# roljon/Steered-Mixture-of-Experts

Hardware: NVIDIA B200
Metric: pixel_kernel_evals_per_s_fwd_bwd (higher is better)
Workload: dtype f32

## Files before the change

### include/smoe_b200.h

```cpp
#ifndef SMOE_B200_H
#define SMOE_B200_H

#include <stddef.h>
#include <stdint.h>

#ifdef __cplusplus
extern "C" {
#endif

#define SMOE_ABI_VERSION 4
#define SMOE_TPIX 512
#define SMOE_NSCAL 16

#define SMOE_PIXEL_ABSENT (-1.0f)
#define SMOE_PIXEL_HALO   (-2.0f)

#define SMOE_E_BADARG (-1)
#define SMOE_E_UNSUPPORTED (-2)

typedef struct smoe_cfg {
    int32_t d;
    int32_t C;
    int32_t precision;
    float   margin;
    int32_t use_determinant;
// ... 56 lines not shown
                  uint8_t* infl_clear , int K_all, void* stream);

int smoe_spatial_keys(const float* centres, int K, int d, int row_stride, const float* grid ,
                      const float* scale , long long* keys, void* stream);

int smoe_forward(const smoe_cfg* cfg, const smoe_batch* batch, const float* packed, const int32_t* indices,
                 const int32_t* counts, const float* chunk_bounds, int K_cap, const float* loss_weights,
                 const float* ax0, const float* ax1, const float* ax2, float* rbuf, int32_t* argmax, uint8_t* infl,
                 float* pix, float* tile_qmin , unsigned long long* pair_counts, void* stream);

int smoe_loss_partials(const smoe_batch* batch);
int smoe_loss(const smoe_cfg* cfg, const smoe_batch* batch, const float* rbuf, const float* image,
              const uint8_t* image_u8, const float* loss_weights, float* res, float* pix, float* scalars,
              float* partials, int32_t* ticket, void* stream);

int smoe_cotangent(const smoe_cfg* cfg, const smoe_batch* batch, const float* rbuf, const float* grad_r, float* pix,
                   void* stream);

int smoe_backward(const smoe_cfg* cfg, const smoe_batch* batch, const float* packed, const int32_t* counts,
                  int K_cap, const float* pix, const float* tile_qmin,
                  const float* ax0, const float* ax1, const float* ax2, int num_splits, float* raw_part,
                  int32_t* plan ,
                  unsigned long long* pair_counts , void* stream);
size_t smoe_backward_plan_bytes(int K_cap, const smoe_batch* batch);
int smoe_suggest_splits(int K_cap, const smoe_batch* batch);

int smoe_reduce_splits(const smoe_cfg* cfg, const int32_t* counts, int K_cap, int num_splits,
                       const float* raw_part, const int32_t* plan ,
                       float* raw, void* stream);

// ... 82 lines not shown
```

### steered-mixture-of-experts_b200/_ffi.py

```python
from __future__ import annotations

import ctypes as C
import os

import torch

_HERE = os.path.dirname(os.path.abspath(__file__))
LIB_PATH = os.path.join(_HERE, "libsmoe_b200.so")

TPIX = 512
ABI_VERSION = 4
NSCAL = 16
STATS_STRIDE = 24

EXPORTS = [
    "smoe_abi_version", "smoe_last_error", "smoe_param_count", "smoe_packed_stride", "smoe_num_tiles", "smoe_pix_stride",
    "smoe_pack_workspace_bytes", "smoe_backward_workspace_bytes", "smoe_backward_plan_bytes", "smoe_pack", "smoe_pack_fed", "smoe_forward", "smoe_loss", "smoe_loss_partials", "smoe_cotangent", "smoe_ssim_loss_workspace_bytes", "smoe_ssim_loss",
    "smoe_backward", "smoe_suggest_splits", "smoe_reduce_splits", "smoe_grad_finalize", "smoe_update_kernel_list",
    "smoe_adam_step", "smoe_step_begin", "smoe_spatial_keys", "smoe_xchg_window_bytes", "smoe_peer_alloc", "smoe_peer_free",
    "smoe_peer_export", "smoe_peer_open", "smoe_peer_close", "smoe_xchg_publish", "smoe_grad_finalize_peers",
    "smoe_xchg_reduce_tail", "smoe_xchg_status", "smoe_feed", "smoe_halo_pull", "smoe_quant_ranges_bytes", "smoe_quant_ranges", "smoe_quant_route", "smoe_fake_quant_theta", "smoe_ssim_workspace_bytes", "smoe_ssim", "smoe_sqerr", "smoe_quantize", "smoe_rescale",
    "smoe_colminmax",
]


class Cfg(C.Structure):
    _fields_ = [("d", C.c_int32), ("C", C.c_int32), ("precision", C.c_int32), ("margin", C.c_float),
                ("use_determinant", C.c_int32), ("train_inverse_cov", C.c_int32), ("use_yuv", C.c_int32),
                ("train_gammas", C.c_int32), ("only_y_gamma", C.c_int32), ("quantize_pis", C.c_int32),
                ("pis_lb", C.c_float), ("pis_ub", C.c_float), ("pis_bits", C.c_int32),
                ("quantization_mode", C.c_int32), ("q_lb", C.c_float * 5), ("q_ub", C.c_float * 5),
                ("q_bits", C.c_int32 * 5), ("use_diff_center", C.c_int32), ("kernel_count_as_norm_l1", C.c_int32),
# ... 76 lines not shown
```

### steered-mixture-of-experts_b200/csrc/forward.cu

```cuda
#include "smoe_common.cuh"

namespace smoe {

template <int D, int C>
struct Rec {
    static constexpr int T = tri(D);
    static constexpr int GN = T + D + 1;
    static constexpr int EN = C + D * C;
    static constexpr int RC0 = (GN + EN + 1 + 3) / 4 * 4;
    static constexpr int RC = (RC0 / 4) % 2 == 0 ? RC0 + 4 : RC0;
    static constexpr int NG4 = (GN + 3) / 4;
    static constexpr int OQ = 0, OL = T, OC = T + D, ONU = GN, OGA = GN + C, OK = GN + EN;
};

template <int D, int C>
__device__ __forceinline__ void transform_record(const float* __restrict__ raw, const float (&mu)[D],
                                                 const float (&ctr)[3], int korig, float* __restrict__ dst) {
    using R = Rec<D, C>;
    float out[R::RC];
    float Qm[D][D], v[D];
#pragma unroll
    for (int l = 0; l < D; ++l)
#pragma unroll
        for (int m = l; m < D; ++m) Qm[l][m] = Qm[m][l] = raw[off_A(D, C) + ut(D, l, m)];
// ... 36 lines not shown
__device__ __forceinline__ void parabola(const float* __restrict__ f, const float (&xs)[3], float& c, float& b) {
    using R = Rec<D, C>;
    c = f[R::OC];
#pragma unroll
    for (int l = 1; l < D; ++l) {
        float t = f[R::OL + l];
#pragma unroll
        for (int m = l; m < D; ++m) t = fmaf(f[R::OQ + ut(D, l, m)], xs[m], t);
        c = fmaf(t, xs[l], c);
    }
    b = f[R::OL + 0];
#pragma unroll
    for (int m = 1; m < D; ++m) b = fmaf(f[R::OQ + ut(D, 0, m)], xs[m], b);
}

struct FwdArgs {
    smoe_cfg cfg;
    smoe_batch b;
    const float* packed;
    const int32_t* indices;
    const int32_t* counts;
    const float* chunk_bounds;
    const float* lossw;
    const float* ax[3];
    float* rbuf;
    int32_t* argmax;
    uint8_t* infl;
    float* pix;
    float* tile_qmin;
    unsigned long long* pair_counts;
    int ntiles, nt1, nt2, max_chunks;
    float tau, ltau;
    float eps_cut;
// ... 16 lines not shown
    *total = tot;
    return off + __popc(bal & ((1u << lane) - 1u));
}

#ifndef SMOE_FWD_CTAS_2D
#define SMOE_FWD_CTAS_2D 6
#endif
#ifndef SMOE_FWD_UNROLL
#define SMOE_FWD_UNROLL 2
#endif
constexpr int kBodyUnroll = SMOE_FWD_UNROLL;
#ifndef SMOE_FWD_NEARCUT
#define SMOE_FWD_NEARCUT 8.0f
#endif
constexpr float kNearCut = SMOE_FWD_NEARCUT;
template <int D, int C, bool COUNT, bool AMAX>
__global__ void __launch_bounds__(kThreadsF, (D == 2) ? SMOE_FWD_CTAS_2D : 4) forward_kernel(const FwdArgs a) {
    using R = Rec<D, C>;
    constexpr int PK = pstride(D, C);
    constexpr int PPT = kPixPerThread;
    static_assert(kChunk == kThreadsF, "one kernel of a chunk per thread");
    extern __shared__ __align__(128) unsigned char smem_raw[];
    float* raw0 = reinterpret_cast<float*>(smem_raw);
    float* raw1 = raw0 + kChunk * PK;
    float* crec = raw1 + kChunk * PK;
    uint64_t* bar = reinterpret_cast<uint64_t*>(crec + kChunk * R::RC);
    float* red = reinterpret_cast<float*>(bar + 2);
    int* scratch = reinterpret_cast<int*>(red + 32);
    int* clist = scratch + 8;

    const int tid = threadIdx.x;
    const int K = a.counts[0];
    const int nchunks = (K + kChunk - 1) / kChunk;
    const int mode = a.cfg.dense_exec;
    const bool cull = mode == 0, skip = mode != 1;
    if (tid == 0) {
        mbar_init(&bar[0], 1);
        mbar_init(&bar[1], 1);
        fence_barrier_init();
    }
    __syncthreads();
    uint32_t phase0 = 0, phase1 = 0;
    int par = 0;
// ... 33 lines not shown
            auto in_halo = [&](int ax, int g) {
                const int o = a.b.origin[ax], e = o + a.b.extent[ax];
                return ax < D && ((o > 0 && g < o + a.b.halo) || (e < a.b.dims[ax] && g >= e - a.b.halo));
            };
            const bool h12 = a.b.halo > 0 && (in_halo(1, g1) || in_halo(2, g2));
            if (D > 1) xs[1] = a.ax[1][min(g1, hi[1])] - ctr[1];
            if (D > 2) xs[2] = a.ax[2][min(g2, hi[2])] - ctr[2];
#pragma unroll
            for (int p = 0; p < PPT; ++p) {
                const int j = p * kThreadsF + tid;
                const int i0 = j / (e2 * e1);
                const int g0 = lo[0] + i0;
                const bool ok = g0 <= hi[0] && g1 <= hi[1] && g2 <= hi[2];
                bool fed = ok;
                if (a.lossw && ok && a.lossw[g0 * a.b.dims[1] * a.b.dims[2] + gbase12] == SMOE_PIXEL_ABSENT) fed = false;
                if (fed) okmask |= 1u << p;
                if (a.b.halo > 0 && (h12 || in_halo(0, g0))) hmask |= 1u << p;
                x0[p] = a.ax[0][min(g0, hi[0])] - ctr[0];
            }
        }

        auto build_chunk_list = [&](float thr, int part) -> int {
            int n = 0;
            for (int base = 0; base < nchunks; base += kThreadsF) {
                const int ci = base + tid;
                bool need = false;
                if (ci < nchunks) {
                    const float* cb = a.chunk_bounds + (size_t)ci * kCB;
                    float d2 = 0.f, kd = 0.f;
#pragma unroll
// ... 182 lines not shown
                    }
#pragma unroll
                    for (int p = 0; p < PPT; ++p) {
                        const float w = ex2f(q[p]);
                        const bool pass = q[p] > ltau;
                        const float wm = pass ? w : 0.f;
#pragma unroll
                        for (int c = 0; c < C; ++c) r[p][c] = fmaf(wm, fmaf(f[R::OGA + c], x0[p], Eb[c]), r[p][c]);
                        if (AMAX && pass && (w > bestw[p] || (w == bestw[p] && korig < bestk[p]))) { bestw[p] = w; bestk[p] = korig; }
                    }
                    if (any && a.infl) a.infl[korig] = 1;
                }
            });
        }

#pragma unroll
        for (int p = 0; p < PPT; ++p) {
            const int j = p * kThreadsF + tid;
            const bool inb = (okmask >> p) & 1u;
            const int gpix = (lo[0] + j / (e2 * e1)) * a.b.dims[1] * a.b.dims[2] + gbase12;
            const bool halo = ((hmask >> p) & 1u) || (a.lossw && inb && a.lossw[gpix] == SMOE_PIXEL_HALO);
            if (inb && !halo) {
#pragma unroll
                for (int c = 0; c < C; ++c) a.rbuf[(size_t)gpix * C + c] = r[p][c];
                if (AMAX) a.argmax[gpix] = bestk[p];
            }
            if (a.pix) {
                const int RLf = a.b.tile[D - 1];
                float* tp = a.pix + (size_t)tile * pix_stride(D, C, RLf);
                tp[PL_Z * SMOE_TPIX + j] = D == 1 ? x0[p] : xs[D - 1];
                tp[PL_QTHR * SMOE_TPIX + j] = inb ? qthr[p] : INFINITY;
                tp[PL_GR * SMOE_TPIX + j] = (inb && ((live_mask >> p) & 1u)) ? 1.f : 0.f;
                if (D > 1 && j % RLf == 0) {
                    const int row = j / RLf, nrows = SMOE_TPIX / RLf;
                    tp[pix_rowc_offset(C) + row] = x0[p];
#pragma unroll
                    for (int l = 1; l < D - 1; ++l) tp[pix_rowc_offset(C) + l * nrows + row] = xs[l];
                }
            }
        }
    }

    if (COUNT) {
        unsigned long long v[4] = {cntA_vis, cntA_ex, cntB_vis, cntB_ex};
#pragma unroll
        for (int q = 0; q < 4; ++q) {
#pragma unroll
            for (int o = 16; o > 0; o >>= 1) v[q] += __shfl_down_sync(0xffffffffu, v[q], o);
            if ((tid & 31) == 0) atomicAdd(&a.pair_counts[q], v[q]);
        }
    }

}

struct LossArgs {
    smoe_cfg cfg;
    smoe_batch b;
    const float* rbuf;
    const float* image;
    const uint8_t* image_u8;
    const float* lossw;
    float* res;
    float* pix;
    float* scalars;
    float* partials;
    int32_t* ticket;
    int ntiles, nt1, nt2, pix_tstride;
    float eps, q_scale, q_inv_scale;
};

template <int C>
__global__ void __launch_bounds__(256) loss_kernel(const LossArgs a) {
    const int tid = threadIdx.x;
    const int e1 = a.b.tile[1], e2 = a.b.tile[2];
    const int D = a.cfg.d;
    float lsum[C];
#pragma unroll
    for (int c = 0; c < C; ++c) lsum[c] = 0.f;
    float sqsum = 0.f;
    int nonfinite = 0;
    {
        int tt[3], lo[3], hi[3];
        tt[0] = blockIdx.y;
        tt[1] = a.nt2 == 1 ? (int)blockIdx.x : (int)blockIdx.x / a.nt2;
        tt[2] = a.nt2 == 1 ? 0 : (int)blockIdx.x % a.nt2;
        const int tile = (tt[0] * a.nt1 + tt[1]) * a.nt2 + tt[2];
#pragma unroll
        for (int i = 0; i < 3; ++i) {
            lo[i] = a.b.origin[i] + tt[i] * a.b.tile[i];
            hi[i] = min(lo[i] + a.b.tile[i], a.b.origin[i] + a.b.extent[i]) - 1;
        }
        auto in_halo = [&](int ax, int g) {
            const int o = a.b.origin[ax], e = o + a.b.extent[ax];
            return ax < D && ((o > 0 && g < o + a.b.halo) || (e < a.b.dims[ax] && g >= e - a.b.halo));
        };
// ... 2 lines not shown
        const int g1 = lo[1] + i1, g2 = lo[2] + i2;
        const bool in12 = g1 <= hi[1] && g2 <= hi[2];
        const bool halo12 = a.b.halo > 0 && (in_halo(1, g1) || in_halo(2, g2));
        const int rows_per_pass = 256 / (e1 * e2);
        int g0 = lo[0] + tid / (e1 * e2);
        for (int j = tid; j < SMOE_TPIX; j += 256, g0 += rows_per_pass) {
            bool inb = in12 && g0 <= hi[0];
            const int gpix = inb ? (g0 * a.b.dims[1] + g1) * a.b.dims[2] + g2 : 0;
            const float lwv = (a.lossw && inb) ? a.lossw[gpix] : 1.f;
            if (lwv == SMOE_PIXEL_ABSENT) inb = false;
            const bool halo = lwv == SMOE_PIXEL_HALO || halo12 || (a.b.halo > 0 && in_halo(0, g0));
            float g[C], gr = 0.f;
#pragma unroll
            for (int c = 0; c < C; ++c) g[c] = 0.f;
            if (inb && !halo) {
#pragma unroll
                for (int c = 0; c < C; ++c) {
                    const size_t gi = (size_t)gpix * C + c;
                    const float rv = a.rbuf[gi];
                    if (!(fabsf(rv) <= 3.0e38f)) nonfinite = 1;
                    const float rc = fminf(fmaxf(rv, 0.f), 1.f);
                    const float kq = floorf(__fadd_rn(__fmul_rn(rc, a.q_inv_scale), 0.5f));
                    const float rq = __fmul_rn(kq, a.q_scale);
                    const float tgt = a.image_u8 ? __fdiv_rn((float)a.image_u8[gi], 255.0f) : a.image[gi];
                    const float diff = __fsub_rn(rq, tgt);
                    const float ad = fabsf(diff) - a.eps;
                    sqsum = fmaf(diff, diff, sqsum);
                    lsum[c] = a.lossw ? fmaf(ad * ad, lwv, lsum[c]) : fmaf(ad, ad, lsum[c]);
                    const float cw = a.cfg.use_yuv ? (c == 0 ? 0.75f : 0.125f) : (1.0f / C);
                    const float sgn = diff > 0.f ? 1.f : (diff < 0.f ? -1.f : 0.f);
                    const bool ste = (rv >= 0.f) && (rv <= 1.f);
                    g[c] = ste ? 2.f * ad * sgn * cw * a.b.inv_count : 0.f;
                    if (a.lossw) g[c] *= lwv;
                    gr = fmaf(g[c], rv, gr);
                    if (a.res) a.res[gi] = rq;
                }
            }
            if (tp) {
                const bool live = tp[PL_GR * SMOE_TPIX + j] != 0.f;
                tp[PL_GR * SMOE_TPIX + j] = live ? gr : 0.f;
#pragma unroll
                for (int c = 0; c < C; ++c) tp[(PL_G + c) * SMOE_TPIX + j] = g[c];
            }
        }
    }
    __shared__ float red[8][8];
    __shared__ float tree[256];
    __shared__ int s_last;
    const int nblk = gridDim.x * gridDim.y, bid = blockIdx.y * gridDim.x + blockIdx.x;
    float vals[8];
#pragma unroll
    for (int q = 0; q < 8; ++q) vals[q] = 0.f;
#pragma unroll
    for (int c = 0; c < C; ++c) vals[c] = lsum[c];
    vals[4] = sqsum;
    vals[5] = (float)nonfinite;
#pragma unroll
    for (int q = 0; q < 6; ++q)
#pragma unroll
        for (int o = 16; o > 0; o >>= 1) vals[q] += __shfl_down_sync(0xffffffffu, vals[q], o);
    if ((tid & 31) == 0)
#pragma unroll
        for (int q = 0; q < 8; ++q) red[tid >> 5][q] = vals[q];
    __syncthreads();
    if (tid < 8) {
        float s = 0.f;
        for (int wv = 0; wv < 8; ++wv) s += red[wv][tid];
        a.partials[(size_t)bid * 8 + tid] = s;
    }
    __threadfence();
    __syncthreads();
    if (tid == 0) s_last = (atomicAdd(a.ticket, 1) == nblk - 1);
    __syncthreads();
    if (s_last) {
        __threadfence();
        for (int q = 0; q < 6; ++q) {
            float s = 0.f;
            for (int bq = tid; bq < nblk; bq += 256) s += __ldcg(&a.partials[(size_t)bq * 8 + q]);
            tree[tid] = s;
            __syncthreads();
            for (int o = 128; o > 0; o >>= 1) {
                if (tid < o) tree[tid] += tree[tid + o];
                __syncthreads();
            }
            if (tid == 0) a.scalars[q] += tree[0];
            __syncthreads();
        }
        if (tid == 0) *a.ticket = 0;
    }
}

struct CotArgs {
    smoe_batch b;
    const float* rbuf;
    const float* grad_r;
    float* pix;
    int nt1, nt2, pix_tstride;
};

template <int C>
__global__ void __launch_bounds__(256) cotangent_kernel(const CotArgs a) {
    const int tid = threadIdx.x;
    const int e1 = a.b.tile[1], e2 = a.b.tile[2];
// ... 24 lines not shown
            for (int c = 0; c < C; ++c) {
                const size_t gi = (size_t)gpix * C + c;
                g[c] = a.grad_r[gi];
                gr = fmaf(g[c], a.rbuf[gi], gr);
            }
        }
        const bool live = tp[PL_GR * SMOE_TPIX + j] != 0.f;
        tp[PL_GR * SMOE_TPIX + j] = live ? gr : 0.f;
#pragma unroll
        for (int c = 0; c < C; ++c) tp[(PL_G + c) * SMOE_TPIX + j] = g[c];
    }
}

template <int D, int C>
static size_t fwd_smem_bytes(int max_chunks) {
    return (size_t)(2 * kChunk * pstride(D, C) + kChunk * Rec<D, C>::RC) * 4 + 2 * 8 + 32 * 4 + 8 * 4 +
           (size_t)max_chunks * 4 + 64;
}

}

using namespace smoe;

extern "C" int smoe_forward(const smoe_cfg* cfg, const smoe_batch* batch, const float* packed, const int32_t* indices,
                            const int32_t* counts, const float* chunk_bounds, int K_cap, const float* loss_weights,
                            const float* ax0, const float* ax1, const float* ax2, float* rbuf, int32_t* argmax,
                            uint8_t* infl, float* pix, float* tile_qmin, unsigned long long* pair_counts, void* stream) {
    SMOE_REQUIRE(cfg && batch && packed && indices && counts && chunk_bounds && ax0 && ax1 && rbuf, "null argument");
    SMOE_REQUIRE(K_cap > 0, "K_cap must be positive");
    SMOE_REQUIRE(cfg->d == 2 || ax2, "ax2 required for d == 3");
    SMOE_REQUIRE(batch->tile[0] * batch->tile[1] * batch->tile[2] == SMOE_TPIX, "tile product must be SMOE_TPIX");
    SMOE_REQUIRE(kThreadsF % (batch->tile[1] * batch->tile[2]) == 0 && batch->tile[cfg->d - 1] % 4 == 0,
                 "tile[1]*tile[2] must divide 128 and the last tile extent must be a multiple of 4");
    SMOE_REQUIRE(!pix || tile_qmin, "tile_qmin is required with pix");
    SMOE_REQUIRE(batch->halo >= 0, "negative halo");
    SMOE_REQUIRE(cfg->eps_bits == 0 || (cfg->eps_bits >= 24 && cfg->eps_bits <= 126), "eps_bits must be 0 or in [24, 126]");
    SMOE_REQUIRE(cfg->eps_bits == 0 || cfg->dense_exec == 0, "eps_bits needs dense_exec == 0");
    for (int i = 0; i < 3; ++i)
        SMOE_REQUIRE(batch->extent[i] > 0 && batch->origin[i] >= 0 && batch->origin[i] + batch->extent[i] <= batch->dims[i],
                     "batch rectangle outside the image");
    SMOE_REQUIRE(cfg->d == 3 || (batch->dims[2] == 1 && batch->tile[2] == 1), "d == 2 needs dims[2] == tile[2] == 1");
    SMOE_REQUIRE((long long)batch->dims[0] * batch->dims[1] * batch->dims[2] < (1ll << 31), "more than 2^31 pixels");
// ... 6 lines not shown
    a.rbuf = rbuf; a.argmax = argmax; a.infl = infl; a.pix = pix; a.tile_qmin = tile_qmin;
    a.pair_counts = pair_counts;
    a.nt1 = (batch->extent[1] + batch->tile[1] - 1) / batch->tile[1];
    a.nt2 = (batch->extent[2] + batch->tile[2] - 1) / batch->tile[2];
    a.ntiles = smoe_num_tiles(batch);
    a.max_chunks = (K_cap + kChunk - 1) / kChunk;
    const float two_p = (float)(1 << cfg->precision);
    a.tau = 0.5f / two_p;
    a.ltau = -(float)(cfg->precision + 1);
    a.eps_cut = (float)cfg->eps_bits;
    int dev = 0, sms = 0;
    cudaGetDevice(&dev);
    cudaDeviceGetAttribute(&sms, cudaDevAttrMultiProcessorCount, dev);
    const int per_sm = cfg->d == 2 ? SMOE_FWD_CTAS_2D : 4;
    int grid = a.ntiles < per_sm * sms ? a.ntiles : per_sm * sms;
    cudaStream_t st = (cudaStream_t)stream;
#define LAUNCH(D, C, CNT, AM)                                                                                       \
    {                                                                                                               \
        size_t sm = fwd_smem_bytes<D, C>(a.max_chunks);                                                             \
        SMOE_REQUIRE(sm <= 200 * 1024, "too many kernel chunks for the shared-memory chunk list");                  \
        cudaFuncSetAttribute(forward_kernel<D, C, CNT, AM>, cudaFuncAttributeMaxDynamicSharedMemorySize, (int)sm);  \
        forward_kernel<D, C, CNT, AM><<<grid, kThreadsF, sm, st>>>(a);                                              \
    }
#define CALL(D, C)                                                               \
    if (pair_counts) { if (argmax) LAUNCH(D, C, true, true) else LAUNCH(D, C, true, false) } \
    else { if (argmax) LAUNCH(D, C, false, true) else LAUNCH(D, C, false, false) }
    SMOE_DISPATCH_DC(cfg->d, cfg->C, CALL)
#undef CALL
#undef LAUNCH
    return check_launch("smoe_forward");
}

extern "C" int smoe_loss_partials(const smoe_batch* batch) {
    return batch ? smoe_num_tiles(batch) : 0;
}

extern "C" int smoe_loss(const smoe_cfg* cfg, const smoe_batch* batch, const float* rbuf, const float* image,
                         const uint8_t* image_u8, const float* loss_weights, float* res, float* pix, float* scalars,
                         float* partials, int32_t* ticket, void* stream) {
    SMOE_REQUIRE(cfg && batch && rbuf && scalars && partials && ticket, "null argument");
    SMOE_REQUIRE((image != nullptr) != (image_u8 != nullptr), "exactly one of image / image_u8");
    SMOE_REQUIRE(batch->tile[0] * batch->tile[1] * batch->tile[2] == SMOE_TPIX, "tile product must be SMOE_TPIX");
    SMOE_REQUIRE(cfg->C == 1 || cfg->C == 3, "1 or 3 channels");
    SMOE_REQUIRE(256 % (batch->tile[1] * batch->tile[2]) == 0, "tile[1]*tile[2] must divide 256");
    LossArgs a;
    a.cfg = *cfg;
    a.b = *batch;
    a.rbuf = rbuf; a.image = image; a.image_u8 = image_u8; a.lossw = loss_weights; a.res = res; a.pix = pix;
    a.scalars = scalars; a.partials = partials; a.ticket = ticket;
    a.nt1 = (batch->extent[1] + batch->tile[1] - 1) / batch->tile[1];
    a.nt2 = (batch->extent[2] + batch->tile[2] - 1) / batch->tile[2];
    a.ntiles = smoe_num_tiles(batch);
    a.pix_tstride = pix_stride(cfg->d, cfg->C, batch->tile[cfg->d - 1]);
    const float two_p = (float)(1 << cfg->precision);
    a.eps = cfg->margin / two_p;
    a.q_scale = 1.0f / (two_p - 1.0f);
    a.q_inv_scale = 1.0f / a.q_scale;
    const int nt0 = a.ntiles / (a.nt1 * a.nt2);
    SMOE_REQUIRE(nt0 <= 65535, "too many tiles along the first axis");
    const dim3 grid(a.nt1 * a.nt2, nt0);
    if (cfg->C == 1) loss_kernel<1><<<grid, 256, 0, (cudaStream_t)stream>>>(a);
    else loss_kernel<3><<<grid, 256, 0, (cudaStream_t)stream>>>(a);
    return check_launch("smoe_loss");
}

extern "C" int smoe_cotangent(const smoe_cfg* cfg, const smoe_batch* batch, const float* rbuf, const float* grad_r,
                              float* pix, void* stream) {
    SMOE_REQUIRE(cfg && batch && rbuf && grad_r && pix, "null argument");
    SMOE_REQUIRE(batch->tile[0] * batch->tile[1] * batch->tile[2] == SMOE_TPIX, "tile product must be SMOE_TPIX");
    SMOE_REQUIRE(batch->halo == 0, "halo must be 0: the cotangent covers the whole batch rectangle");
    SMOE_REQUIRE((cfg->d == 2 || cfg->d == 3) && (cfg->C == 1 || cfg->C == 3), "d in {2, 3} and 1 or 3 channels");
    SMOE_REQUIRE(256 % (batch->tile[1] * batch->tile[2]) == 0, "tile[1]*tile[2] must divide 256");
// ... 14 lines not shown
```

### steered-mixture-of-experts_b200/csrc/smoe_common.cuh

```cuda
#pragma once
#include <cuda_runtime.h>
#include <stdint.h>
#include <stdio.h>
#include <math.h>
#include "../../include/smoe_b200.h"

#if defined(__CUDA_ARCH__) && (__CUDA_ARCH__ < 1000)
#error "libsmoe_b200 is written for sm_100a (B200) only"
#endif

namespace smoe {

#ifndef SMOE_BWD_THREADS
#define SMOE_BWD_THREADS 64
#endif
#ifndef SMOE_BWD_HALVES
#define SMOE_BWD_HALVES 2
#endif
constexpr int kThreads = SMOE_BWD_THREADS;
constexpr int kHalves = SMOE_BWD_HALVES;
constexpr int kGroup = kThreads / kHalves;
constexpr int kFin = 64;
constexpr int kThreadsF = 128;
constexpr int kPixPerThread = SMOE_TPIX / kThreadsF;
// ... 92 lines not shown
    for (int sp = 0; sp < used; sp += 8) {
        float v[8];
#pragma unroll
        for (int u = 0; u < 8; ++u) v[u] = (sp + u < used) ? p[(size_t)(sp + u) * stride] : 0.f;
#pragma unroll
        for (int u = 0; u < 8; ++u)
            if (sp + u < used) acc += v[u];
    }
    return acc;
}
__device__ __forceinline__ float ex2f(float x) {
    float y;
    asm("ex2.approx.ftz.f32 %0, %1;" : "=f"(y) : "f"(x));
    return y;
}
__device__ __forceinline__ uint32_t smem_u32(const void* p) {
    return (uint32_t)__cvta_generic_to_shared(p);
}
__device__ __forceinline__ void mbar_init(uint64_t* bar, uint32_t count) {
    asm volatile("mbarrier.init.shared::cta.b64 [%0], %1;" ::"r"(smem_u32(bar)), "r"(count));
}
__device__ __forceinline__ void fence_barrier_init() {
    asm volatile("fence.mbarrier_init.release.cluster;" ::: "memory");
}
__device__ __forceinline__ void fence_proxy_async() {
    asm volatile("fence.proxy.async.shared::cta;" ::: "memory");
}
__device__ __forceinline__ void mbar_expect_tx(uint64_t* bar, uint32_t bytes) {
    asm volatile("mbarrier.arrive.expect_tx.shared::cta.b64 _, [%0], %1;" ::"r"(smem_u32(bar)), "r"(bytes)
                 : "memory");
// ... 25 lines not shown
```

### steered-mixture-of-experts_b200/smoe.py

```python
from __future__ import annotations

import ctypes as C
import math
from itertools import product

import numpy as np
import torch

import os
import warnings

from . import _ffi
from ._ffi import Adam, Batch, Cfg, Peers, check, lib, ptr, stream_ptr
from .quantizer import quantize_params, rescaler

PARAM_KEYS = ("pis", "musX", "A_diagonal", "A_corr", "gamma_e", "nu_e")


def theta_offsets(d, C):
    T = d * (d + 1) // 2
    return dict(mu=0, A=d, pi=d + T, nu=d + T + 1, ga=d + T + 1 + C)


def a_col(d, l, m):
# ... 683 lines not shown
                self._graphs[key] = "warm"
            else:
                if state == "warm":
                    l0 = self.gpu_launches
                    if self._img_pending:
                        torch.cuda.current_stream().wait_event(self._img_event)
                        self._img_pending = False
                    torch.cuda.synchronize()
                    try:
                        graphs = []
                        for phase in (("pre", "post") if len(self._batches) == 1 else ()):
                            g = torch.cuda.CUDAGraph()
                            with torch.cuda.graph(g):
                                self._enqueue(pis_l1, u_l1, True, False, False, lossw=lossw, phase=phase)
                            graphs.append(g)
                        gall = torch.cuda.CUDAGraph()
                        with torch.cuda.graph(gall):
                            self._enqueue(pis_l1, u_l1, True, False, False, lossw=lossw)
                        state = (gall, graphs, (self.gpu_launches - l0) // (2 if graphs else 1))
                    except Exception as exc:
                        if os.environ.get("SMOE_ALLOW_EAGER", "0") != "1":
                            raise RuntimeError(f"smoe_b200: CUDA graph capture of the training step failed ({exc}); "
                                               "set SMOE_ALLOW_EAGER=1 to run the step eagerly instead") from exc
                        warnings.warn(f"smoe_b200: CUDA graph capture failed ({exc}); running eagerly")
                        self.use_cuda_graphs = False
                        torch.cuda.synchronize()
                        state = None
                    self.gpu_launches = l0
                    if state is not None:
                        self._graphs[key] = state
                if state is not None:
                    if self._img_pending and state[1]:
                        state[1][0].replay()
                        torch.cuda.current_stream().wait_event(self._img_event)
                        self._img_pending = False
                        state[1][1].replay()
                    else:
                        if self._img_pending:
                            torch.cuda.current_stream().wait_event(self._img_event)
                            self._img_pending = False
                        state[0].replay()
                    self.gpu_launches += state[2]
                    replayed = True
        if not replayed:
            self._enqueue(pis_l1, u_l1, train, update_reconstruction, with_quantized_params,
                          lossw=lossw, batches=batches)
        torch.cuda.current_stream().synchronize()
        h = self._host_f32.tolist()
        hi = self._host_i32.tolist()
        for row, irow in zip(h, hi):
            row[_ffi.NSCAL:_ffi.NSCAL + 4] = irow[_ffi.NSCAL:_ffi.NSCAL + 4]
        norm = float(self.start_pis)
        Cc = self.image.shape[-1]
        loss_val = mse_val = 0.0
        num_pi = -1
        for ii, b in enumerate(batches):
            inv_n = float(b.inv_count)
# ... 101 lines not shown
            rp = {k: torch.as_tensor(np.ascontiguousarray(np.asarray(v, dtype=np.float32)), device=self.device)
                  for k, v in self.rparams.items()}
            Kf = int(rp["pis"].shape[0])
            if Kf > K:
                raise ValueError("more fed kernels than model kernels")
            fkeys = torch.empty((Kf,), dtype=torch.int64, device=self.device)
            check(L.smoe_spatial_keys(ptr(rp["musX"]), Kf, self.dim_domain, self.dim_domain, ptr(None), self._key_scale,
                                      ptr(fkeys), st), "smoe_spatial_keys")
            forder = torch.sort(fkeys, stable=True).indices.to(torch.int32)
        norm = float(self.start_pis)
        if pre and self._qdyn is not None and not fed:
            check(L.smoe_quant_ranges(C.byref(self._cfg), ptr(self._theta), K, int(self.train_musx), ptr(self._qdyn), st),
                  "smoe_quant_ranges")
            self.gpu_launches += 2
        ax2 = ptr(self._d_axes[2]) if self.dim_domain == 3 else ptr(None)
        for ii, b in enumerate(batches):
            counts, regs, scal = self._counts[ii], self._regsums[ii], self._scalars[ii]
            tq = self._tile_qmin[ii]
            if pre:
                if fed:
                    check(L.smoe_pack_fed(C.byref(self._cfg), ptr(rp["A"]), ptr(rp["musX"]), ptr(rp["nu_e"]),
                                          ptr(rp["gamma_e"]), ptr(rp["pis"]), ptr(forder), Kf, ptr(self._packed),
                                          ptr(self._indices), ptr(counts), ptr(self._chunk_bounds), ptr(scal),
                                          ptr(self._infl), K, st), "smoe_pack_fed")
                    regs.zero_()
                    self.gpu_launches += 3
                else:
                    check(L.smoe_pack(C.byref(self._cfg), ptr(self._theta), ptr(self._mus_grid), ptr(self._qdyn),
                                      ptr(self._klist[ii]), ptr(self._perm), K, ptr(self._packed),
                                      ptr(self._indices), ptr(self._pos), ptr(counts), ptr(regs), ptr(self._chunk_bounds),
                                      ptr(self._pack_ws), ptr(self._grads) if (train and ii == 0) else ptr(None),
                                      ptr(scal), ptr(self._infl), st), "smoe_pack")
                    self.gpu_launches += 3
                check(L.smoe_forward(C.byref(self._cfg), C.byref(b), ptr(self._packed), ptr(self._indices), ptr(counts),
                                     ptr(self._chunk_bounds), K, ptr(lossw), ptr(self._d_axes[0]), ptr(self._d_axes[1]),
                                     ax2, ptr(self._d_res_pre), ptr(self._d_argmax) if update_reconstruction else ptr(None),
                                     ptr(self._infl), ptr(self._pix) if train else ptr(None), ptr(tq), pc, st),
                      "smoe_forward")
                self.gpu_launches += 1
                if self._batch_phantom[ii]:
                    pb, halo1 = self._phantom
                    check(L.smoe_forward(C.byref(self._cfg), C.byref(pb), ptr(self._packed), ptr(self._indices),
                                         ptr(counts), ptr(self._chunk_bounds), K, ptr(halo1), ptr(self._d_axes[0]),
                                         ptr(self._d_axes[1]), ax2, ptr(self._d_res_pre), ptr(None), ptr(self._infl),
                                         ptr(None), ptr(None), ptr(None), st), "smoe_forward (phantom)")
                    self.gpu_launches += 1
            if not post:
                continue
            if phase == "all" and self._img_pending:
                torch.cuda.current_stream().wait_event(self._img_event)
                self._img_pending = False
            check(L.smoe_loss(C.byref(self._cfg), C.byref(b), ptr(self._d_res_pre),
                              ptr(None) if self._use_u8 else ptr(self._d_image),
                              ptr(self._d_image_u8) if self._use_u8 else ptr(None), ptr(lossw),
                              ptr(self._d_res) if (update_reconstruction or self.ssim_opt or not train) else ptr(None),
                              ptr(self._pix) if train else ptr(None), ptr(scal), ptr(self._partials), ptr(self._ticket),
                              st), "smoe_loss")
            self.gpu_launches += 1
            if self.ssim_opt:
                if self._halo is not None:
                    check(L.smoe_halo_pull(C.byref(self._peers), C.byref(self._halo), st), "smoe_halo_pull")
                    self.gpu_launches += 1
                check(L.smoe_ssim_loss(C.byref(self._cfg), C.byref(b),
                                       C.byref(self._ssim_region) if self._ssim_region is not None else ptr(None),
                                       ptr(self._d_res), ptr(self._d_image),
                                       ptr(self._d_res_pre), ptr(self._pix) if train else ptr(None), ptr(scal),
                                       ptr(self._ssim_ws), st), "smoe_ssim_loss")
                self.gpu_launches += 2 * self.dim_domain + 2 if train else self.dim_domain + 1
            if train:
                check(L.smoe_backward(C.byref(self._cfg), C.byref(b), ptr(self._packed), ptr(counts), K,
                                      ptr(self._pix), ptr(tq), ptr(self._d_axes[0]), ptr(self._d_axes[1]), ax2,
                                      self._splits, ptr(self._raw_part), ptr(self._plan), pc, st), "smoe_backward")
                self.gpu_launches += 2
# ... 468 lines not shown
```

Baseline: 83300 billion.

## Fuse loss computation into forward kernel epilogue with last-block reduction

Adds a LOSS template variant of the forward kernel that computes the quantized loss, per-pixel gradients and per-tile partial sums in its epilogue. The final cross-tile reduction is done by the last block to finish, using a ticket. Target pixels are prefetched into L2 early in the tile. Python uses the fused entry point whenever the phase is 'all' and no SSIM, phantom batch or pending image is involved, which removes a separate loss launch and a re-read of rbuf. The cost is more registers and an extra grid-wide reduction tail in the forward kernel, which may hurt its occupancy.

```diff
diff --git a/include/smoe_b200.h b/include/smoe_b200.h
--- a/include/smoe_b200.h
+++ b/include/smoe_b200.h
@@ -8,7 +8,7 @@
 extern "C" {
 #endif
 
-#define SMOE_ABI_VERSION 4
+#define SMOE_ABI_VERSION 5
 #define SMOE_TPIX 512
 #define SMOE_NSCAL 16
 
@@ -95,6 +95,13 @@
               const uint8_t* image_u8, const float* loss_weights, float* res, float* pix, float* scalars,
               float* partials, int32_t* ticket, void* stream);
 
+int smoe_forward_loss(const smoe_cfg* cfg, const smoe_batch* batch, const float* packed, const int32_t* indices,
+                      const int32_t* counts, const float* chunk_bounds, int K_cap, const float* loss_weights,
+                      const float* ax0, const float* ax1, const float* ax2, float* rbuf, int32_t* argmax, uint8_t* infl,
+                      float* pix, float* tile_qmin , unsigned long long* pair_counts, const float* image,
+                      const uint8_t* image_u8, float* res, float* scalars, float* partials, int32_t* ticket,
+                      void* stream);
+
 int smoe_cotangent(const smoe_cfg* cfg, const smoe_batch* batch, const float* rbuf, const float* grad_r, float* pix,
                    void* stream);
 
diff --git a/steered-mixture-of-experts_b200/_ffi.py b/steered-mixture-of-experts_b200/_ffi.py
--- a/steered-mixture-of-experts_b200/_ffi.py
+++ b/steered-mixture-of-experts_b200/_ffi.py
@@ -9,13 +9,13 @@
 LIB_PATH = os.path.join(_HERE, "libsmoe_b200.so")
 
 TPIX = 512
-ABI_VERSION = 4
+ABI_VERSION = 5
 NSCAL = 16
 STATS_STRIDE = 24
 
 EXPORTS = [
     "smoe_abi_version", "smoe_last_error", "smoe_param_count", "smoe_packed_stride", "smoe_num_tiles", "smoe_pix_stride",
-    "smoe_pack_workspace_bytes", "smoe_backward_workspace_bytes", "smoe_backward_plan_bytes", "smoe_pack", "smoe_pack_fed", "smoe_forward", "smoe_loss", "smoe_loss_partials", "smoe_cotangent", "smoe_ssim_loss_workspace_bytes", "smoe_ssim_loss",
+    "smoe_pack_workspace_bytes", "smoe_backward_workspace_bytes", "smoe_backward_plan_bytes", "smoe_pack", "smoe_pack_fed", "smoe_forward", "smoe_forward_loss", "smoe_loss", "smoe_loss_partials", "smoe_cotangent", "smoe_ssim_loss_workspace_bytes", "smoe_ssim_loss",
     "smoe_backward", "smoe_suggest_splits", "smoe_reduce_splits", "smoe_grad_finalize", "smoe_update_kernel_list",
     "smoe_adam_step", "smoe_step_begin", "smoe_spatial_keys", "smoe_xchg_window_bytes", "smoe_peer_alloc", "smoe_peer_free",
     "smoe_peer_export", "smoe_peer_open", "smoe_peer_close", "smoe_xchg_publish", "smoe_grad_finalize_peers",
diff --git a/steered-mixture-of-experts_b200/csrc/forward.cu b/steered-mixture-of-experts_b200/csrc/forward.cu
--- a/steered-mixture-of-experts_b200/csrc/forward.cu
+++ b/steered-mixture-of-experts_b200/csrc/forward.cu
@@ -74,9 +74,70 @@
     for (int m = 1; m < D; ++m) b = fmaf(f[R::OQ + ut(D, 0, m)], xs[m], b);
 }
 
+struct LossIO {
+    const float* image;
+    const uint8_t* image_u8;
+    float* res;
+    float* scalars;
+    float* partials;
+    int32_t* ticket;
+    float eps, q_scale, q_inv_scale;
+};
+
+template <int C>
+struct LossAcc {
+    float lsum[C];
+    float sqsum;
+};
+
+__device__ __forceinline__ float load_target(const LossIO& io, size_t gi) {
+    return io.image_u8 ? __fdiv_rn((float)io.image_u8[gi], 255.0f) : io.image[gi];
+}
+
+template <int C>
+__device__ __forceinline__ void pixel_loss(const LossIO& io, bool use_yuv, float inv_count, bool weighted, float lwv,
+                                           int gpix, const float (&rv)[C], const float (&tgt)[C], LossAcc<C>& acc,
+                                           unsigned& nonfinite, unsigned nfbit, float (&g)[C], float& gr) {
+    gr = 0.f;
+#pragma unroll
+    for (int c = 0; c < C; ++c) {
+        const size_t gi = (size_t)gpix * C + c;
+        if (!(fabsf(rv[c]) <= 3.0e38f)) nonfinite |= nfbit;
+        const float rc = fminf(fmaxf(rv[c], 0.f), 1.f);
+        const float kq = floorf(__fadd_rn(__fmul_rn(rc, io.q_inv_scale), 0.5f));
+        const float rq = __fmul_rn(kq, io.q_scale);
+        const float diff = __fsub_rn(rq, tgt[c]);
+        const float ad = fabsf(diff) - io.eps;
+        acc.sqsum = fmaf(diff, diff, acc.sqsum);
+        acc.lsum[c] = weighted ? fmaf(ad * ad, lwv, acc.lsum[c]) : fmaf(ad, ad, acc.lsum[c]);
+        const float cw = use_yuv ? (c == 0 ? 0.75f : 0.125f) : (1.0f / C);
+        const float sgn = diff > 0.f ? 1.f : (diff < 0.f ? -1.f : 0.f);
+        const bool ste = (rv[c] >= 0.f) && (rv[c] <= 1.f);
+        g[c] = ste ? 2.f * ad * sgn * cw * inv_count : 0.f;
+        if (weighted) g[c] *= lwv;
+        gr = fmaf(g[c], rv[c], gr);
+        if (io.res) io.res[gi] = rq;
+    }
+}
+
+template <int C>
+__device__ __forceinline__ void loss_vals(const LossAcc<C>& acc, unsigned nonfinite, float (&vals)[8]) {
+#pragma unroll
+    for (int q = 0; q < 8; ++q) vals[q] = 0.f;
+#pragma unroll
+    for (int c = 0; c < C; ++c) vals[c] = acc.lsum[c];
+    vals[4] = acc.sqsum;
+    vals[5] = (float)nonfinite;
+#pragma unroll
+    for (int q = 0; q < 6; ++q)
+#pragma unroll
+        for (int o = 16; o > 0; o >>= 1) vals[q] += __shfl_down_sync(0xffffffffu, vals[q], o);
+}
+
 struct FwdArgs {
     smoe_cfg cfg;
     smoe_batch b;
+    LossIO io;
     const float* packed;
     const int32_t* indices;
     const int32_t* counts;
@@ -123,7 +184,7 @@
 #define SMOE_FWD_NEARCUT 8.0f
 #endif
 constexpr float kNearCut = SMOE_FWD_NEARCUT;
-template <int D, int C, bool COUNT, bool AMAX>
+template <int D, int C, bool COUNT, bool AMAX, bool LOSS>
 __global__ void __launch_bounds__(kThreadsF, (D == 2) ? SMOE_FWD_CTAS_2D : 4) forward_kernel(const FwdArgs a) {
     using R = Rec<D, C>;
     constexpr int PK = pstride(D, C);
@@ -135,7 +196,7 @@
     float* crec = raw1 + kChunk * PK;
     uint64_t* bar = reinterpret_cast<uint64_t*>(crec + kChunk * R::RC);
     float* red = reinterpret_cast<float*>(bar + 2);
-    int* scratch = reinterpret_cast<int*>(red + 32);
+    int* scratch = reinterpret_cast<int*>(red + 64);
     int* clist = scratch + 8;
 
     const int tid = threadIdx.x;
@@ -199,6 +260,10 @@
                 const bool ok = g0 <= hi[0] && g1 <= hi[1] && g2 <= hi[2];
                 bool fed = ok;
                 if (a.lossw && ok && a.lossw[g0 * a.b.dims[1] * a.b.dims[2] + gbase12] == SMOE_PIXEL_ABSENT) fed = false;
+                if (LOSS && ok) {
+                    const size_t gi = (size_t)(g0 * a.b.dims[1] * a.b.dims[2] + gbase12) * C;
+                    prefetch_l2(a.io.image_u8 ? (const void*)(a.io.image_u8 + gi) : (const void*)(a.io.image + gi));
+                }
                 if (fed) okmask |= 1u << p;
                 if (a.b.halo > 0 && (h12 || in_halo(0, g0))) hmask |= 1u << p;
                 x0[p] = a.ax[0][min(g0, hi[0])] - ctr[0];
@@ -411,23 +476,56 @@
             });
         }
 
+        static_assert(!LOSS || PPT == 4, "the LOSS epilogue maps 4 pixels per thread onto 2 loss_kernel threads");
+        LossAcc<C> acc[2];
+        unsigned nonfinite = 0;
+        float tg[LOSS ? PPT : 1][C];
+        if (LOSS) {
+#pragma unroll
+            for (int p = 0; p < PPT; ++p) {
+                const int gpix = (lo[0] + (p * kThreadsF + tid) / (e2 * e1)) * a.b.dims[1] * a.b.dims[2] + gbase12;
+#pragma unroll
+                for (int c = 0; c < C; ++c) tg[p][c] = ((okmask >> p) & 1u) ? load_target(a.io, (size_t)gpix * C + c) : 0.f;
+            }
+        }
+        if (LOSS) {
+#pragma unroll
+            for (int h = 0; h < 2; ++h) {
+#pragma unroll
+                for (int c = 0; c < C; ++c) acc[h].lsum[c] = 0.f;
+                acc[h].sqsum = 0.f;
+            }
+        }
 #pragma unroll
         for (int p = 0; p < PPT; ++p) {
             const int j = p * kThreadsF + tid;
             const bool inb = (okmask >> p) & 1u;
             const int gpix = (lo[0] + j / (e2 * e1)) * a.b.dims[1] * a.b.dims[2] + gbase12;
-            const bool halo = ((hmask >> p) & 1u) || (a.lossw && inb && a.lossw[gpix] == SMOE_PIXEL_HALO);
+            const float lwv = (a.lossw && inb) ? a.lossw[gpix] : 1.f;
+            const bool halo = ((hmask >> p) & 1u) || lwv == SMOE_PIXEL_HALO;
+            float g[C], gr = 0.f;
+#pragma unroll
+            for (int c = 0; c < C; ++c) g[c] = 0.f;
             if (inb && !halo) {
 #pragma unroll
                 for (int c = 0; c < C; ++c) a.rbuf[(size_t)gpix * C + c] = r[p][c];
                 if (AMAX) a.argmax[gpix] = bestk[p];
+                if (LOSS) pixel_loss<C>(a.io, a.cfg.use_yuv, a.b.inv_count, a.lossw != nullptr, lwv, gpix, r[p],
+                                        tg[p], acc[p & 1], nonfinite, 1u << (p & 1), g, gr);
             }
             if (a.pix) {
                 const int RLf = a.b.tile[D - 1];
                 float* tp = a.pix + (size_t)tile * pix_stride(D, C, RLf);
+                const bool live = inb && ((live_mask >> p) & 1u);
                 tp[PL_Z * SMOE_TPIX + j] = D == 1 ? x0[p] : xs[D - 1];
                 tp[PL_QTHR * SMOE_TPIX + j] = inb ? qthr[p] : INFINITY;
-                tp[PL_GR * SMOE_TPIX + j] = (inb && ((live_mask >> p) & 1u)) ? 1.f : 0.f;
+                if (LOSS) {
+                    tp[PL_GR * SMOE_TPIX + j] = live ? gr : 0.f;
+#pragma unroll
+                    for (int c = 0; c < C; ++c) tp[(PL_G + c) * SMOE_TPIX + j] = g[c];
+                } else {
+                    tp[PL_GR * SMOE_TPIX + j] = live ? 1.f : 0.f;
+                }
                 if (D > 1 && j % RLf == 0) {
                     const int row = j / RLf, nrows = SMOE_TPIX / RLf;
                     tp[pix_rowc_offset(C) + row] = x0[p];
@@ -436,6 +534,77 @@
                 }
             }
         }
+        if (LOSS) {
+#pragma unroll
+            for (int h = 0; h < 2; ++h) {
+                float vals[8];
+                loss_vals<C>(acc[h], (nonfinite >> h) & 1u, vals);
+                if ((tid & 31) == 0)
+#pragma unroll
+                    for (int q = 0; q < 8; ++q) red[((tid >> 5) + 4 * h) * 8 + q] = vals[q];
+            }
+            __syncthreads();
+            if (tid < 8) {
+                float s = 0.f;
+                for (int wv = 0; wv < 8; ++wv) s += red[wv * 8 + tid];
+                a.io.partials[(size_t)tile * 8 + tid] = s;
+            }
+        }
+    }
+
+    if (LOSS) {
+        __threadfence();
+        __syncthreads();
+        const int last = __syncthreads_or(tid == 0 && atomicAdd(a.io.ticket, 1) == (int)gridDim.x - 1);
+        if (last) {
+            __threadfence();
+            static_assert(kChunk * R::RC >= 6 * kThreadsF, "the trees live in crec");
+            float* tree = crec;
+            constexpr int U = 4;
+            float s0[6], s1[6];
+#pragma unroll
+            for (int q = 0; q < 6; ++q) s0[q] = s1[q] = 0.f;
+            for (int base = tid; base < a.ntiles; base += U * 2 * kThreadsF) {
+                float v[U][2][6];
+#pragma unroll
+                for (int u = 0; u < U; ++u)
+#pragma unroll
+                    for (int h = 0; h < 2; ++h) {
+                        const int bq = base + (2 * u + h) * kThreadsF;
+                        float4 x = make_float4(0.f, 0.f, 0.f, 0.f);
+                        float2 y = make_float2(0.f, 0.f);
+                        if (bq < a.ntiles) {
+                            x = __ldcg(reinterpret_cast<const float4*>(a.io.partials + (size_t)bq * 8));
+                            y = __ldcg(reinterpret_cast<const float2*>(a.io.partials + (size_t)bq * 8 + 4));
+                        }
+                        v[u][h][0] = x.x; v[u][h][1] = x.y; v[u][h][2] = x.z; v[u][h][3] = x.w;
+                        v[u][h][4] = y.x; v[u][h][5] = y.y;
+                    }
+#pragma unroll
+                for (int u = 0; u < U; ++u) {
+                    const int bq = base + 2 * u * kThreadsF;
+#pragma unroll
+                    for (int q = 0; q < 6; ++q) {
+                        if (bq < a.ntiles) s0[q] += v[u][0][q];
+                        if (bq + kThreadsF < a.ntiles) s1[q] += v[u][1][q];
+                    }
+                }
+            }
+#pragma unroll
+            for (int q = 0; q < 6; ++q) tree[q * kThreadsF + tid] = s0[q] + s1[q];
+            __syncthreads();
+            for (int o = kThreadsF / 2; o > 0; o >>= 1) {
+                if (tid < o)
+#pragma unroll
+                    for (int q = 0; q < 6; ++q) tree[q * kThreadsF + tid] += tree[q * kThreadsF + tid + o];
+                __syncthreads();
+            }
+            if (tid == 0) {
+#pragma unroll
+                for (int q = 0; q < 6; ++q) a.io.scalars[q] += tree[q * kThreadsF];
+                *a.io.ticket = 0;
+            }
+        }
     }
 
     if (COUNT) {
@@ -453,17 +622,11 @@
 struct LossArgs {
     smoe_cfg cfg;
     smoe_batch b;
+    LossIO io;
     const float* rbuf;
-    const float* image;
-    const uint8_t* image_u8;
     const float* lossw;
-    float* res;
     float* pix;
-    float* scalars;
-    float* partials;
-    int32_t* ticket;
     int ntiles, nt1, nt2, pix_tstride;
-    float eps, q_scale, q_inv_scale;
 };
 
 template <int C>
@@ -471,11 +634,11 @@
     const int tid = threadIdx.x;
     const int e1 = a.b.tile[1], e2 = a.b.tile[2];
     const int D = a.cfg.d;
-    float lsum[C];
-#pragma unroll
-    for (int c = 0; c < C; ++c) lsum[c] = 0.f;
-    float sqsum = 0.f;
-    int nonfinite = 0;
+    LossAcc<C> acc;
+#pragma unroll
+    for (int c = 0; c < C; ++c) acc.lsum[c] = 0.f;
+    acc.sqsum = 0.f;
+    unsigned nonfinite = 0;
     {
         int tt[3], lo[3], hi[3];
         tt[0] = blockIdx.y;
@@ -508,27 +671,14 @@
 #pragma unroll
             for (int c = 0; c < C; ++c) g[c] = 0.f;
             if (inb && !halo) {
+                float rv[C], tg[C];
 #pragma unroll
                 for (int c = 0; c < C; ++c) {
-                    const size_t gi = (size_t)gpix * C + c;
-                    const float rv = a.rbuf[gi];
-                    if (!(fabsf(rv) <= 3.0e38f)) nonfinite = 1;
-                    const float rc = fminf(fmaxf(rv, 0.f), 1.f);
-                    const float kq = floorf(__fadd_rn(__fmul_rn(rc, a.q_inv_scale), 0.5f));
-                    const float rq = __fmul_rn(kq, a.q_scale);
-                    const float tgt = a.image_u8 ? __fdiv_rn((float)a.image_u8[gi], 255.0f) : a.image[gi];
-                    const float diff = __fsub_rn(rq, tgt);
-                    const float ad = fabsf(diff) - a.eps;
-                    sqsum = fmaf(diff, diff, sqsum);
-                    lsum[c] = a.lossw ? fmaf(ad * ad, lwv, lsum[c]) : fmaf(ad, ad, lsum[c]);
-                    const float cw = a.cfg.use_yuv ? (c == 0 ? 0.75f : 0.125f) : (1.0f / C);
-                    const float sgn = diff > 0.f ? 1.f : (diff < 0.f ? -1.f : 0.f);
-                    const bool ste = (rv >= 0.f) && (rv <= 1.f);
-                    g[c] = ste ? 2.f * ad * sgn * cw * a.b.inv_count : 0.f;
-                    if (a.lossw) g[c] *= lwv;
-                    gr = fmaf(g[c], rv, gr);
-                    if (a.res) a.res[gi] = rq;
-                }
+                    rv[c] = a.rbuf[(size_t)gpix * C + c];
+                    tg[c] = load_target(a.io, (size_t)gpix * C + c);
+                }
+                pixel_loss<C>(a.io, a.cfg.use_yuv, a.b.inv_count, a.lossw != nullptr, lwv, gpix, rv, tg, acc, nonfinite,
+                              1u, g, gr);
             }
             if (tp) {
                 const bool live = tp[PL_GR * SMOE_TPIX + j] != 0.f;
@@ -543,16 +693,7 @@
     __shared__ int s_last;
     const int nblk = gridDim.x * gridDim.y, bid = blockIdx.y * gridDim.x + blockIdx.x;
     float vals[8];
-#pragma unroll
-    for (int q = 0; q < 8; ++q) vals[q] = 0.f;
-#pragma unroll
-    for (int c = 0; c < C; ++c) vals[c] = lsum[c];
-    vals[4] = sqsum;
-    vals[5] = (float)nonfinite;
-#pragma unroll
-    for (int q = 0; q < 6; ++q)
-#pragma unroll
-        for (int o = 16; o > 0; o >>= 1) vals[q] += __shfl_down_sync(0xffffffffu, vals[q], o);
+    loss_vals<C>(acc, nonfinite, vals);
     if ((tid & 31) == 0)
 #pragma unroll
         for (int q = 0; q < 8; ++q) red[tid >> 5][q] = vals[q];
@@ -560,27 +701,27 @@
     if (tid < 8) {
         float s = 0.f;
         for (int wv = 0; wv < 8; ++wv) s += red[wv][tid];
-        a.partials[(size_t)bid * 8 + tid] = s;
+        a.io.partials[(size_t)bid * 8 + tid] = s;
     }
     __threadfence();
     __syncthreads();
-    if (tid == 0) s_last = (atomicAdd(a.ticket, 1) == nblk - 1);
+    if (tid == 0) s_last = (atomicAdd(a.io.ticket, 1) == nblk - 1);
     __syncthreads();
     if (s_last) {
         __threadfence();
         for (int q = 0; q < 6; ++q) {
             float s = 0.f;
-            for (int bq = tid; bq < nblk; bq += 256) s += __ldcg(&a.partials[(size_t)bq * 8 + q]);
+            for (int bq = tid; bq < nblk; bq += 256) s += __ldcg(&a.io.partials[(size_t)bq * 8 + q]);
             tree[tid] = s;
             __syncthreads();
             for (int o = 128; o > 0; o >>= 1) {
                 if (tid < o) tree[tid] += tree[tid + o];
                 __syncthreads();
             }
-            if (tid == 0) a.scalars[q] += tree[0];
+            if (tid == 0) a.io.scalars[q] += tree[0];
             __syncthreads();
         }
-        if (tid == 0) *a.ticket = 0;
+        if (tid == 0) *a.io.ticket = 0;
     }
 }
 
@@ -635,7 +776,7 @@
 
 template <int D, int C>
 static size_t fwd_smem_bytes(int max_chunks) {
-    return (size_t)(2 * kChunk * pstride(D, C) + kChunk * Rec<D, C>::RC) * 4 + 2 * 8 + 32 * 4 + 8 * 4 +
+    return (size_t)(2 * kChunk * pstride(D, C) + kChunk * Rec<D, C>::RC) * 4 + 2 * 8 + 64 * 4 + 8 * 4 +
            (size_t)max_chunks * 4 + 64;
 }
 
@@ -643,10 +784,23 @@
 
 using namespace smoe;
 
-extern "C" int smoe_forward(const smoe_cfg* cfg, const smoe_batch* batch, const float* packed, const int32_t* indices,
-                            const int32_t* counts, const float* chunk_bounds, int K_cap, const float* loss_weights,
-                            const float* ax0, const float* ax1, const float* ax2, float* rbuf, int32_t* argmax,
-                            uint8_t* infl, float* pix, float* tile_qmin, unsigned long long* pair_counts, void* stream) {
+static LossIO loss_io(const smoe_cfg* cfg, const float* image, const uint8_t* image_u8, float* res, float* scalars,
+                      float* partials, int32_t* ticket) {
+    LossIO io;
+    io.image = image; io.image_u8 = image_u8; io.res = res;
+    io.scalars = scalars; io.partials = partials; io.ticket = ticket;
+    const float two_p = (float)(1 << cfg->precision);
+    io.eps = cfg->margin / two_p;
+    io.q_scale = 1.0f / (two_p - 1.0f);
+    io.q_inv_scale = 1.0f / io.q_scale;
+    return io;
+}
+
+static int smoe_forward_impl(const smoe_cfg* cfg, const smoe_batch* batch, const float* packed, const int32_t* indices,
+                             const int32_t* counts, const float* chunk_bounds, int K_cap, const float* loss_weights,
+                             const float* ax0, const float* ax1, const float* ax2, float* rbuf, int32_t* argmax,
+                             uint8_t* infl, float* pix, float* tile_qmin, unsigned long long* pair_counts,
+                             const LossIO* io, void* stream) {
     SMOE_REQUIRE(cfg && batch && packed && indices && counts && chunk_bounds && ax0 && ax1 && rbuf, "null argument");
     SMOE_REQUIRE(K_cap > 0, "K_cap must be positive");
     SMOE_REQUIRE(cfg->d == 2 || ax2, "ax2 required for d == 3");
@@ -683,21 +837,47 @@
     cudaDeviceGetAttribute(&sms, cudaDevAttrMultiProcessorCount, dev);
     const int per_sm = cfg->d == 2 ? SMOE_FWD_CTAS_2D : 4;
     int grid = a.ntiles < per_sm * sms ? a.ntiles : per_sm * sms;
+    a.io = io ? *io : LossIO{};
     cudaStream_t st = (cudaStream_t)stream;
-#define LAUNCH(D, C, CNT, AM)                                                                                       \
-    {                                                                                                               \
-        size_t sm = fwd_smem_bytes<D, C>(a.max_chunks);                                                             \
-        SMOE_REQUIRE(sm <= 200 * 1024, "too many kernel chunks for the shared-memory chunk list");                  \
-        cudaFuncSetAttribute(forward_kernel<D, C, CNT, AM>, cudaFuncAttributeMaxDynamicSharedMemorySize, (int)sm);  \
-        forward_kernel<D, C, CNT, AM><<<grid, kThreadsF, sm, st>>>(a);                                              \
-    }
-#define CALL(D, C)                                                               \
-    if (pair_counts) { if (argmax) LAUNCH(D, C, true, true) else LAUNCH(D, C, true, false) } \
-    else { if (argmax) LAUNCH(D, C, false, true) else LAUNCH(D, C, false, false) }
+#define LAUNCH(D, C, CNT, AM, LS)                                                                                      \
+    {                                                                                                                  \
+        size_t sm = fwd_smem_bytes<D, C>(a.max_chunks);                                                                \
+        SMOE_REQUIRE(sm <= 200 * 1024, "too many kernel chunks for the shared-memory chunk list");                     \
+        cudaFuncSetAttribute(forward_kernel<D, C, CNT, AM, LS>, cudaFuncAttributeMaxDynamicSharedMemorySize, (int)sm); \
+        forward_kernel<D, C, CNT, AM, LS><<<grid, kThreadsF, sm, st>>>(a);                                             \
+    }
+#define CALL_LS(D, C, LS)                                                                        \
+    if (pair_counts) { if (argmax) LAUNCH(D, C, true, true, LS) else LAUNCH(D, C, true, false, LS) } \
+    else { if (argmax) LAUNCH(D, C, false, true, LS) else LAUNCH(D, C, false, false, LS) }
+#define CALL(D, C) \
+    if (io) { CALL_LS(D, C, true) } else { CALL_LS(D, C, false) }
     SMOE_DISPATCH_DC(cfg->d, cfg->C, CALL)
 #undef CALL
+#undef CALL_LS
 #undef LAUNCH
-    return check_launch("smoe_forward");
+    return check_launch(io ? "smoe_forward_loss" : "smoe_forward");
+}
+
+extern "C" int smoe_forward(const smoe_cfg* cfg, const smoe_batch* batch, const float* packed, const int32_t* indices,
+                            const int32_t* counts, const float* chunk_bounds, int K_cap, const float* loss_weights,
+                            const float* ax0, const float* ax1, const float* ax2, float* rbuf, int32_t* argmax,
+                            uint8_t* infl, float* pix, float* tile_qmin, unsigned long long* pair_counts, void* stream) {
+    return smoe_forward_impl(cfg, batch, packed, indices, counts, chunk_bounds, K_cap, loss_weights, ax0, ax1, ax2, rbuf,
+                             argmax, infl, pix, tile_qmin, pair_counts, nullptr, stream);
+}
+
+extern "C" int smoe_forward_loss(const smoe_cfg* cfg, const smoe_batch* batch, const float* packed,
+                                 const int32_t* indices, const int32_t* counts, const float* chunk_bounds, int K_cap,
+                                 const float* loss_weights, const float* ax0, const float* ax1, const float* ax2,
+                                 float* rbuf, int32_t* argmax, uint8_t* infl, float* pix, float* tile_qmin,
+                                 unsigned long long* pair_counts, const float* image, const uint8_t* image_u8,
+                                 float* res, float* scalars, float* partials, int32_t* ticket, void* stream) {
+    SMOE_REQUIRE(cfg && scalars && partials && ticket, "null argument");
+    SMOE_REQUIRE((image != nullptr) != (image_u8 != nullptr), "exactly one of image / image_u8");
+    SMOE_REQUIRE(((uintptr_t)partials & 15) == 0, "partials must be 16-byte aligned");
+    const LossIO io = loss_io(cfg, image, image_u8, res, scalars, partials, ticket);
+    return smoe_forward_impl(cfg, batch, packed, indices, counts, chunk_bounds, K_cap, loss_weights, ax0, ax1, ax2, rbuf,
+                             argmax, infl, pix, tile_qmin, pair_counts, &io, stream);
 }
 
 extern "C" int smoe_loss_partials(const smoe_batch* batch) {
@@ -715,16 +895,12 @@
     LossArgs a;
     a.cfg = *cfg;
     a.b = *batch;
-    a.rbuf = rbuf; a.image = image; a.image_u8 = image_u8; a.lossw = loss_weights; a.res = res; a.pix = pix;
-    a.scalars = scalars; a.partials = partials; a.ticket = ticket;
+    a.io = loss_io(cfg, image, image_u8, res, scalars, partials, ticket);
+    a.rbuf = rbuf; a.lossw = loss_weights; a.pix = pix;
     a.nt1 = (batch->extent[1] + batch->tile[1] - 1) / batch->tile[1];
     a.nt2 = (batch->extent[2] + batch->tile[2] - 1) / batch->tile[2];
     a.ntiles = smoe_num_tiles(batch);
     a.pix_tstride = pix_stride(cfg->d, cfg->C, batch->tile[cfg->d - 1]);
-    const float two_p = (float)(1 << cfg->precision);
-    a.eps = cfg->margin / two_p;
-    a.q_scale = 1.0f / (two_p - 1.0f);
-    a.q_inv_scale = 1.0f / a.q_scale;
     const int nt0 = a.ntiles / (a.nt1 * a.nt2);
     SMOE_REQUIRE(nt0 <= 65535, "too many tiles along the first axis");
     const dim3 grid(a.nt1 * a.nt2, nt0);
diff --git a/steered-mixture-of-experts_b200/csrc/smoe_common.cuh b/steered-mixture-of-experts_b200/csrc/smoe_common.cuh
--- a/steered-mixture-of-experts_b200/csrc/smoe_common.cuh
+++ b/steered-mixture-of-experts_b200/csrc/smoe_common.cuh
@@ -130,6 +130,9 @@
     asm("ex2.approx.ftz.f32 %0, %1;" : "=f"(y) : "f"(x));
     return y;
 }
+__device__ __forceinline__ void prefetch_l2(const void* p) {
+    asm volatile("prefetch.L2 [%0];" ::"l"(p));
+}
 __device__ __forceinline__ uint32_t smem_u32(const void* p) {
     return (uint32_t)__cvta_generic_to_shared(p);
 }
diff --git a/steered-mixture-of-experts_b200/smoe.py b/steered-mixture-of-experts_b200/smoe.py
--- a/steered-mixture-of-experts_b200/smoe.py
+++ b/steered-mixture-of-experts_b200/smoe.py
@@ -721,10 +721,11 @@
                             with torch.cuda.graph(g):
                                 self._enqueue(pis_l1, u_l1, True, False, False, lossw=lossw, phase=phase)
                             graphs.append(g)
+                        l1 = self.gpu_launches
                         gall = torch.cuda.CUDAGraph()
                         with torch.cuda.graph(gall):
                             self._enqueue(pis_l1, u_l1, True, False, False, lossw=lossw)
-                        state = (gall, graphs, (self.gpu_launches - l0) // (2 if graphs else 1))
+                        state = (gall, graphs, self.gpu_launches - l1, l1 - l0)
                     except Exception as exc:
                         if os.environ.get("SMOE_ALLOW_EAGER", "0") != "1":
                             raise RuntimeError(f"smoe_b200: CUDA graph capture of the training step failed ({exc}); "
@@ -742,12 +743,13 @@
                         torch.cuda.current_stream().wait_event(self._img_event)
                         self._img_pending = False
                         state[1][1].replay()
+                        self.gpu_launches += state[3]
                     else:
                         if self._img_pending:
                             torch.cuda.current_stream().wait_event(self._img_event)
                             self._img_pending = False
                         state[0].replay()
-                    self.gpu_launches += state[2]
+                        self.gpu_launches += state[2]
                     replayed = True
         if not replayed:
             self._enqueue(pis_l1, u_l1, train, update_reconstruction, with_quantized_params,
@@ -879,9 +881,12 @@
                   "smoe_quant_ranges")
             self.gpu_launches += 2
         ax2 = ptr(self._d_axes[2]) if self.dim_domain == 3 else ptr(None)
+        img = (ptr(None), ptr(self._d_image_u8)) if self._use_u8 else (ptr(self._d_image), ptr(None))
+        res = ptr(self._d_res) if (update_reconstruction or self.ssim_opt or not train) else ptr(None)
         for ii, b in enumerate(batches):
             counts, regs, scal = self._counts[ii], self._regsums[ii], self._scalars[ii]
             tq = self._tile_qmin[ii]
+            fused = phase == "all" and not self._img_pending and not self.ssim_opt and not self._batch_phantom[ii]
             if pre:
                 if fed:
                     check(L.smoe_pack_fed(C.byref(self._cfg), ptr(rp["A"]), ptr(rp["musX"]), ptr(rp["nu_e"]),
@@ -897,11 +902,15 @@
                                       ptr(self._pack_ws), ptr(self._grads) if (train and ii == 0) else ptr(None),
                                       ptr(scal), ptr(self._infl), st), "smoe_pack")
                     self.gpu_launches += 3
-                check(L.smoe_forward(C.byref(self._cfg), C.byref(b), ptr(self._packed), ptr(self._indices), ptr(counts),
-                                     ptr(self._chunk_bounds), K, ptr(lossw), ptr(self._d_axes[0]), ptr(self._d_axes[1]),
-                                     ax2, ptr(self._d_res_pre), ptr(self._d_argmax) if update_reconstruction else ptr(None),
-                                     ptr(self._infl), ptr(self._pix) if train else ptr(None), ptr(tq), pc, st),
-                      "smoe_forward")
+                fwd_args = (C.byref(self._cfg), C.byref(b), ptr(self._packed), ptr(self._indices), ptr(counts),
+                            ptr(self._chunk_bounds), K, ptr(lossw), ptr(self._d_axes[0]), ptr(self._d_axes[1]), ax2,
+                            ptr(self._d_res_pre), ptr(self._d_argmax) if update_reconstruction else ptr(None),
+                            ptr(self._infl), ptr(self._pix) if train else ptr(None), ptr(tq), pc)
+                if fused:
+                    check(L.smoe_forward_loss(*fwd_args, *img, res, ptr(scal), ptr(self._partials), ptr(self._ticket),
+                                              st), "smoe_forward_loss")
+                else:
+                    check(L.smoe_forward(*fwd_args, st), "smoe_forward")
                 self.gpu_launches += 1
                 if self._batch_phantom[ii]:
                     pb, halo1 = self._phantom
@@ -915,13 +924,11 @@
             if phase == "all" and self._img_pending:
                 torch.cuda.current_stream().wait_event(self._img_event)
                 self._img_pending = False
-            check(L.smoe_loss(C.byref(self._cfg), C.byref(b), ptr(self._d_res_pre),
-                              ptr(None) if self._use_u8 else ptr(self._d_image),
-                              ptr(self._d_image_u8) if self._use_u8 else ptr(None), ptr(lossw),
-                              ptr(self._d_res) if (update_reconstruction or self.ssim_opt or not train) else ptr(None),
-                              ptr(self._pix) if train else ptr(None), ptr(scal), ptr(self._partials), ptr(self._ticket),
-                              st), "smoe_loss")
-            self.gpu_launches += 1
+            if not fused:
+                check(L.smoe_loss(C.byref(self._cfg), C.byref(b), ptr(self._d_res_pre), *img, ptr(lossw), res,
+                                  ptr(self._pix) if train else ptr(None), ptr(scal), ptr(self._partials),
+                                  ptr(self._ticket), st), "smoe_loss")
+                self.gpu_launches += 1
             if self.ssim_opt:
                 if self._halo is not None:
                     check(L.smoe_halo_pull(C.byref(self._peers), C.byref(self._halo), st), "smoe_halo_pull")
```

Measured after the change: 86160 billion (median of 6 runs). 1.03x the previous value.
